# ZechangSun/QFA

Hardware: AMD Instinct MI355X
Metric: spectra/sec per EM step (higher is better)
Workload: dtype f32

## Files before the change

### qfa_amd/csrc/qfa_common.h

```cpp
#pragma once
#include <hip/hip_runtime.h>
#include <stdint.h>

#include <type_traits>
#include <utility>

#include "../../include/qfa_hip.h"

typedef float f32x4 __attribute__((ext_vector_type(4)));

#define QFA_LOG2PI 1.8378770664093453f
#define QFA_LOG2E 1.4426950408889634f
#define QFA_LN2 0.6931471805599453f

template <int KP>
struct Cfg {
    static constexpr int FW = KP < 16 ? 16 : KP;
    static constexpr int KK2 = KP * (KP + 1) / 2;
    static constexpr int NT = (KK2 + 15) / 16;
    static constexpr int PW = NT * 16;
    static constexpr int NFT = FW / 16;
    static constexpr int PFT_PSI = KP + KK2;
    static constexpr int NR = (KP + KK2 + 5 + 3) / 4 * 4;
    static constexpr bool XS3 = KP == 16 || KP == 32;
    static constexpr int PFT_MAIN = XS3 ? (NR * 16 + 255) / 256 * 256 : NR * 16;
    static constexpr int PFT_FP = XS3 ? (KP == 32 ? 1536 : 512) : 0;
    static constexpr int PFT_F16H = 768, PFT_F16M = 1024, PFT_F16IT = 1280;
    static constexpr int TILE_PFT = PFT_MAIN + PFT_FP;
    static constexpr int NMOM = 2 * PW + 2 * FW + 4;
    static constexpr int MOM_T = PW, MOM_B = 2 * PW, MOM_B2 = 2 * PW + FW, MOM_S = 2 * PW + 2 * FW;
    static constexpr int NSOL = 2 * KP + KK2 + KP * KP;
    static constexpr int SOL_CI = KP, SOL_Z = KP + KK2, SOL_P = KP + KK2 + KP * KP;
};

__host__ __device__ constexpr int pair_index(int a, int b, int KP) {
    return a * KP - (a * (a - 1)) / 2 + (b - a);
}

__host__ __device__ inline int round_up(int x, int m) { return (x + m - 1) / m * m; }

#ifndef QFA_PX_SPW
#define QFA_PX_SPW 2
#endif
#ifndef QFA_PX_SPW8
#define QFA_PX_SPW8 1
#endif
struct WorkPlan {
    int full, rem, nseg, seg_tiles;
    __host__ __device__ int items() const { return full + rem * nseg; }
};
__device__ __forceinline__ void plan_item(const WorkPlan &w, int item, int ntiles, int &blk, int &seg, int &t0,
                                          int &t1) {
    if (item < w.full) {
        blk = item; seg = 0; t0 = 0; t1 = ntiles;
    } else {
        const int j = item - w.full;
        blk = w.full + j % w.rem;
        seg = j / w.rem;
        t0 = seg * w.seg_tiles;
        t1 = min(t0 + w.seg_tiles, ntiles);
    }
}

template <int NMOM>
__device__ __forceinline__ float *mom_segment(float *MOM, const WorkPlan &w, int seg, int Bpad, int spb = 64) {
    if (seg == 0) return MOM;
    const size_t row0 = (size_t)w.full * spb, R = (size_t)Bpad - row0;
    return MOM + ((size_t)Bpad + (size_t)(seg - 1) * R - row0) * NMOM;
}

struct Scal64 {
    double s[3];
    unsigned ticket, pad;
};
__device__ __forceinline__ void scal64_commit(Scal64 *q, double a, double b, double c, unsigned nwaves, float *accS) {
    if ((threadIdx.x & 63) != 0) return;
    if (a != 0.0) atomicAdd(&q->s[0], a);
    if (b != 0.0) atomicAdd(&q->s[1], b);
    if (c != 0.0) atomicAdd(&q->s[2], c);
    __threadfence();
    if (atomicAdd(&q->ticket, 1u) == nwaves - 1u) {
        __threadfence();
        accS[0] += (float)__hip_atomic_load(&q->s[0], __ATOMIC_RELAXED, __HIP_MEMORY_SCOPE_AGENT);
        accS[1] += (float)__hip_atomic_load(&q->s[1], __ATOMIC_RELAXED, __HIP_MEMORY_SCOPE_AGENT);
        accS[2] += (float)__hip_atomic_load(&q->s[2], __ATOMIC_RELAXED, __HIP_MEMORY_SCOPE_AGENT);
    }
}

struct DevConsts {
    float tau0, c0, beta;
    float t_amp, t_lscale, t_expo, t_off;
    float offp, k1, omc0;
};

#ifdef QFA_PRECISE_MATH
__device__ __forceinline__ float fast_exp2(float x) { return exp2f(x); }
__device__ __forceinline__ float fast_log2(float x) { return log2f(x); }
__device__ __forceinline__ float fast_rcp(float x) { return 1.0f / x; }
#else
__device__ __forceinline__ float fast_exp2(float x) { return __builtin_amdgcn_exp2f(x); }
__device__ __forceinline__ float fast_log2(float x) { return __builtin_amdgcn_logf(x); }
__device__ __forceinline__ float fast_rcp(float x) { return __builtin_amdgcn_rcpf(x); }
#endif
__device__ __forceinline__ float fast_exp(float x) { return fast_exp2(x * QFA_LOG2E); }
__device__ __forceinline__ float fast_log(float x) { return fast_log2(x) * QFA_LN2; }

struct BlueTerms {
    float A, zd, pw, l2;
};

__device__ __forceinline__ BlueTerms blue_terms(float z, const DevConsts &k) {
    BlueTerms t;
    t.l2 = fast_log2(1.0f + z);
    float tau = k.t_amp * fast_exp2(k.t_expo * (t.l2 + k.t_lscale)) + k.t_off;
    t.A = fast_exp(-tau);
    t.pw = fast_exp2(k.beta * t.l2);
    float re = 1.0f - k.c0 - fast_exp(-k.tau0 * t.pw);
    t.zd = re * re;
    return t;
}

struct ZFac {
    float ts, pw, l2;
};
__device__ __forceinline__ ZFac zfac_load(const float4 *__restrict__ ZS, int s, bool valid) {
    ZFac z{0.f, 0.f, 0.f};
    if (valid) {
        const float4 q = ZS[s];
        z.ts = q.x; z.pw = q.y; z.l2 = q.z;
    }
    return z;
}
__device__ __forceinline__ BlueTerms blue_terms_zf(const ZFac &zs, float ti, float pwi, float l2i, const DevConsts &k) {
    BlueTerms t;
    t.l2 = zs.l2 + l2i;
    t.pw = zs.pw * pwi;
    t.A = fast_exp2(fmaf(zs.ts, ti, k.offp));
    const float re = k.omc0 - fast_exp2(k.k1 * t.pw);
    t.zd = re * re;
    return t;
}
__device__ __forceinline__ unsigned long long batch_row(const qfa_batch_t &bt, int s) {
    return bt.rows ? (unsigned long long)(unsigned)bt.rows[s] : (unsigned long long)(unsigned)s;
}
template <int SH>
__device__ __forceinline__ const unsigned char *lane_ptr(const void *sbase, unsigned long long off) {
    return reinterpret_cast<const unsigned char *>(sbase) + (off << SH);
}

__device__ __forceinline__ float4 zfac_spec(float zq1, float beta, const qfa_tau_t &tau) {
    const double l2s = log2((double)zq1);
    const double ts = -1.4426950408889634 * (double)tau.amp * exp2((double)tau.expo * (l2s + log2((double)tau.scale)));
    return float4{(float)ts, (float)exp2((double)beta * l2s), (float)l2s, 0.f};
}
__device__ __forceinline__ void zfac_spec_body(int s, const float *__restrict__ zq1, const int *__restrict__ rows,
                                               const qfa_params_t &p, const qfa_tau_t &tau, int B, float4 *__restrict__ ZS) {
    if (s >= B) return;
    ZS[s] = zfac_spec(zq1[rows ? rows[s] : s], *p.beta, tau);
}
static __global__ void k_zfac_spec(const float *__restrict__ zq1, const int *__restrict__ rows, qfa_params_t p, qfa_tau_t tau,
                                   int B, float4 *__restrict__ ZS) {
    zfac_spec_body(blockIdx.x * blockDim.x + threadIdx.x, zq1, rows, p, tau, B, ZS);
}
static __global__ void k_zfac_pix(const float *__restrict__ pix_ratio, qfa_params_t p, qfa_tau_t tau, int Nb,
                                  float4 *__restrict__ ZP) {
    const int i = blockIdx.x * blockDim.x + threadIdx.x;
    if (i >= Nb) return;
    const double l2i = log2((double)pix_ratio[i]);
    ZP[i] = float4{(float)exp2((double)tau.expo * l2i), (float)exp2((double)*p.beta * l2i), (float)l2i, 0.f};
}

struct ZPSrc {
    const float4 *tab;
    const float *ratio;
    const float *beta;
    float expo;
    float offp;
    __device__ __forceinline__ bool on() const { return tab != nullptr || ratio != nullptr; }
    __device__ __forceinline__ float4 at(int i) const {
        if (tab) return tab[i];
        const double l2i = log2((double)ratio[i]);
        return float4{(float)exp2((double)expo * l2i), (float)exp2((double)*beta * l2i), (float)l2i, 0.f};
    }
};
__host__ __device__ inline ZPSrc zp_table(const float4 *ZP, float offp = 0.f) { return ZPSrc{ZP, nullptr, nullptr, 0.f, offp}; }

__device__ __forceinline__ f32x4 mfma4(float a, float b, f32x4 c) {
    return __builtin_amdgcn_mfma_f32_16x16x4f32(a, b, c, 0, 0, 0);
}


typedef unsigned u32x4 __attribute__((ext_vector_type(4)));
typedef unsigned u32x2 __attribute__((ext_vector_type(2)));
typedef __bf16 bf16x8 __attribute__((ext_vector_type(8)));
typedef short s16x4 __attribute__((ext_vector_type(4)));

typedef __bf16 bf16x2 __attribute__((ext_vector_type(2)));
typedef float f32x2v __attribute__((ext_vector_type(2)));
__device__ __forceinline__ unsigned cvt_pk_bf16(float a, float b) {
    return __builtin_bit_cast(unsigned, __builtin_convertvector(f32x2v{a, b}, bf16x2));
}
__device__ __forceinline__ unsigned split_c_lo() {
    unsigned c;
    asm("s_mov_b32 %0, 0xbf80" : "=s"(c));
    return c;
}
__device__ __forceinline__ unsigned split_c_hi() {
    unsigned c;
    asm("s_mov_b32 %0, 0xbf800000" : "=s"(c));
    return c;
}
__device__ __forceinline__ float sub_bf16_lo(float x, unsigned packed) {
    return __builtin_amdgcn_fdot2_f32_bf16(__builtin_bit_cast(bf16x2, packed), __builtin_bit_cast(bf16x2, split_c_lo()), x, false);
}
__device__ __forceinline__ float sub_bf16_hi(float x, unsigned packed) {
    return __builtin_amdgcn_fdot2_f32_bf16(__builtin_bit_cast(bf16x2, packed), __builtin_bit_cast(bf16x2, split_c_hi()), x, false);
}
__device__ __forceinline__ void split2(float x0, float x1, unsigned &h, unsigned &m, unsigned &l) {
    h = cvt_pk_bf16(x0, x1);
    const float r0 = sub_bf16_lo(x0, h), r1 = sub_bf16_hi(x1, h);
    m = cvt_pk_bf16(r0, r1);
    const float s0 = sub_bf16_lo(r0, m), s1 = sub_bf16_hi(r1, m);
    l = cvt_pk_bf16(s0, s1);
}
__device__ __forceinline__ void split8(const float (&x)[8], u32x4 &h, u32x4 &m, u32x4 &l) {
#pragma unroll
    for (int q = 0; q < 4; ++q) {
        unsigned a, b, c;
        split2(x[2 * q], x[2 * q + 1], a, b, c);
        h[q] = a; m[q] = b; l[q] = c;
    }
}
__device__ __forceinline__ f32x4 xdl(const u32x4 &a, const u32x4 &b, f32x4 c) {
    return __builtin_amdgcn_mfma_f32_16x16x32_bf16(__builtin_bit_cast(bf16x8, a), __builtin_bit_cast(bf16x8, b), c, 0,
                                                   0, 0);
}
typedef _Float16 f16x8 __attribute__((ext_vector_type(8)));
typedef _Float16 f16x2 __attribute__((ext_vector_type(2)));
__device__ __forceinline__ void split2h(float x0, float x1, unsigned &h, unsigned &m) {
    const _Float16 h0 = (_Float16)x0, h1 = (_Float16)x1;
    const _Float16 m0 = (_Float16)(x0 - (float)h0), m1 = (_Float16)(x1 - (float)h1);
    h = __builtin_bit_cast(unsigned, f16x2{h0, h1});
    m = __builtin_bit_cast(unsigned, f16x2{m0, m1});
}
__device__ __forceinline__ void split8h(const float (&x)[8], u32x4 &h, u32x4 &m) {
#pragma unroll
    for (int q = 0; q < 4; ++q) {
        unsigned a, b;
        split2h(x[2 * q], x[2 * q + 1], a, b);
        h[q] = a; m[q] = b;
    }
}
__device__ __forceinline__ f32x4 xdlh(const u32x4 &a, const u32x4 &b, f32x4 c) {
    return __builtin_amdgcn_mfma_f32_16x16x32_f16(__builtin_bit_cast(f16x8, a), __builtin_bit_cast(f16x8, b), c, 0, 0, 0);
}
__device__ __forceinline__ f32x4 xdl3h(const u32x4 &ah, const u32x4 &am, const u32x4 &bh, const u32x4 &bm, f32x4 c) {
    c = xdlh(ah, bm, c);
    c = xdlh(am, bh, c);
    return xdlh(ah, bh, c);
}
__host__ __device__ __forceinline__ float f16_row_scale(float amax, float &inv) {
    int e = 0;
    if (amax > 0.f && amax < 3.0e38f) (void)frexpf(amax, &e); else e = 14;
    e = e < -100 ? -100 : (e > 100 ? 100 : e);
    inv = ldexpf(1.f, e - 14);
    return ldexpf(1.f, 14 - e);
}
__host__ __device__ __forceinline__ float f16_weight_scale(float psi) {
    if (!(psi > 0.f && psi < 3.0e38f)) return 0.015625f;
    int e = 0;
    (void)frexpf(psi, &e);
    e = e < -60 ? -60 : (e > 60 ? 60 : e);
    return ldexpf(1.f, 11 + e);
}
__device__ __forceinline__ f32x4 xdl16(const u32x2 &a, const u32x2 &b, f32x4 c) {
    return __builtin_amdgcn_mfma_f32_16x16x16bf16_1k(__builtin_bit_cast(s16x4, a), __builtin_bit_cast(s16x4, b), c, 0,
                                                     0, 0);
}
template <typename V, typename F>
__device__ __forceinline__ f32x4 six_terms(F &&mm, const V &ah, const V &am, const V &al, const V &bh, const V &bm,
                                           const V &bl, f32x4 c) {
    c = mm(ah, bl, c);
    c = mm(al, bh, c);
    c = mm(am, bm, c);
    c = mm(am, bh, c);
    c = mm(ah, bm, c);
    return mm(ah, bh, c);
}
__device__ __forceinline__ f32x4 xdl6(const u32x4 &ah, const u32x4 &am, const u32x4 &al, const u32x4 &bh,
                                      const u32x4 &bm, const u32x4 &bl, f32x4 c) {
    return six_terms([](const u32x4 &a, const u32x4 &b, f32x4 cc) { return xdl(a, b, cc); }, ah, am, al, bh, bm, bl, c);
}
__device__ __forceinline__ f32x4 xdl16_6(const u32x2 &ah, const u32x2 &am, const u32x2 &al, const u32x2 &bh,
                                         const u32x2 &bm, const u32x2 &bl, f32x4 c) {
    return six_terms([](const u32x2 &a, const u32x2 &b, f32x4 cc) { return xdl16(a, b, cc); }, ah, am, al, bh, bm, bl, c);
}

__device__ __forceinline__ void glds16(const void *g, void *lds_base) {
    __builtin_amdgcn_global_load_lds((const __attribute__((address_space(1))) void *)g,
                                     (__attribute__((address_space(3))) void *)lds_base, 16, 0, 0);
}

__device__ __forceinline__ void pin(float &x) { asm volatile("" : "+v"(x)); }
template <typename... T>
__device__ __forceinline__ void pin(float &x, T &...rest) {
    pin(x);
    pin(rest...);
}

__device__ __forceinline__ int dpp_row_bcast(int v, int l) {
#define QFA_BC(n) case n: return __builtin_amdgcn_mov_dpp(v, 0x150 + n, 0xf, 0xf, true);
    switch (l & 15) {
        QFA_BC(0) QFA_BC(1) QFA_BC(2) QFA_BC(3) QFA_BC(4) QFA_BC(5) QFA_BC(6) QFA_BC(7)
        QFA_BC(8) QFA_BC(9) QFA_BC(10) QFA_BC(11) QFA_BC(12) QFA_BC(13) QFA_BC(14) QFA_BC(15)
    }
#undef QFA_BC
    return v;
}
__device__ __forceinline__ int half_bcast(int v, int l) {
    const int a = __builtin_amdgcn_readlane(v, l & 31), b = __builtin_amdgcn_readlane(v, 32 + (l & 31));
    return (threadIdx.x & 32) ? b : a;
}
template <int KP>
__device__ __forceinline__ float group_bcast(float x, int l) {
    if constexpr (KP == 16) return __int_as_float(dpp_row_bcast(__float_as_int(x), l));
    else if constexpr (KP == 32) return __int_as_float(half_bcast(__float_as_int(x), l));
    else return __shfl(x, l, KP);
}
template <int KP>
__device__ __forceinline__ double group_bcast(double x, int l) {
    if constexpr (KP == 16) {
        const int lo = dpp_row_bcast(__double2loint(x), l), hi = dpp_row_bcast(__double2hiint(x), l);
        return __hiloint2double(hi, lo);
    } else if constexpr (KP == 32) {
        const int lo = half_bcast(__double2loint(x), l), hi = half_bcast(__double2hiint(x), l);
        return __hiloint2double(hi, lo);
    } else {
        return __shfl(x, l, KP);
    }
}

template <typename F, int... I>
__device__ __forceinline__ void static_for_impl(F &&f, std::integer_sequence<int, I...>) {
    (f(std::integral_constant<int, I>{}), ...);
}
template <int N, typename F>
__device__ __forceinline__ void static_for(F &&f) {
    static_for_impl(f, std::make_integer_sequence<int, N>{});
}

__device__ __forceinline__ int wave_uniform(int x) { return __builtin_amdgcn_readfirstlane(x); }

__device__ __forceinline__ DevConsts load_consts(const qfa_params_t &p, const qfa_tau_t &tau) {
    DevConsts k;
    k.tau0 = *p.tau0;
    k.c0 = *p.c0;
    k.beta = *p.beta;
    const double l2s = log2((double)tau.scale);
    k.t_lscale = (float)l2s;
    k.t_amp = (float)((double)tau.amp * exp2((double)tau.expo * (l2s - (double)k.t_lscale)));
    k.t_expo = tau.expo;
    k.t_off = tau.offset;
    k.offp = -QFA_LOG2E * k.t_off;
    k.k1 = -QFA_LOG2E * k.tau0;
    k.omc0 = 1.0f - k.c0;
    return k;
}
```

### qfa_amd/csrc/qfa_step_kernels.h

```cpp
#pragma once
#include <type_traits>

#include "qfa_common.h"
#include "qfa_gt_layout.h"

template <int KP>
__global__ void k_prep_pft(const float *__restrict__ F, const float *__restrict__ Psi,
                           const float *__restrict__ omega, const float4 *__restrict__ ZP, int Npix, int Nb, int Nh,
                           int NpixPad, float *__restrict__ PFT) {
    using C = Cfg<KP>;
    const int i = blockIdx.x * blockDim.y + threadIdx.y;
    if (i >= NpixPad) return;
    const bool live = i < Npix;
    float *pft = PFT + (size_t)(i >> 4) * C::TILE_PFT + (i & 15);
    for (int r = threadIdx.x; r < C::NR; r += blockDim.x) {
        float v = 0.f;
        if (r < KP) {
            if (live && r < Nh) v = F[(size_t)i * Nh + r];
        } else if (r < C::PFT_PSI) {
            const int pidx = r - KP;
            int a = 0;
            while (a + 1 < KP && pair_index(a + 1, a + 1, KP) <= pidx) ++a;
            const int b = a + (pidx - pair_index(a, a, KP));
            if (live && b < Nh) v = F[(size_t)i * Nh + a] * F[(size_t)i * Nh + b];
        } else if (r == C::PFT_PSI) {
            if (live) v = Psi[i];
        } else if (r == C::PFT_PSI + 1) {
            if (i < Nb) v = omega[i];
        } else if (ZP && i < Nb && r < C::PFT_PSI + 5) {
            const float4 q = ZP[i];
            v = r == C::PFT_PSI + 2 ? q.x : (r == C::PFT_PSI + 3 ? q.y : q.z);
        }
        pft[r * 16] = v;
    }
    if constexpr (C::XS3 && KP == 32) {
        if (threadIdx.x < 4) {
            const int g = threadIdx.x;
            unsigned *fp = reinterpret_cast<unsigned *>(PFT + (size_t)(i >> 4) * C::TILE_PFT + C::PFT_MAIN) +
                           (g * 16 + (i & 15)) * 4;
#pragma unroll
            for (int q = 0; q < 4; ++q) {
                const int a = 8 * g + 2 * q;
                const float v0 = (live && a < Nh) ? F[(size_t)i * Nh + a] : 0.f;
                const float v1 = (live && a + 1 < Nh) ? F[(size_t)i * Nh + a + 1] : 0.f;
                unsigned h, m, l;
                split2(v0, v1, h, m, l);
                fp[q] = h; fp[256 + q] = m; fp[512 + q] = l;
            }
            float mx = 0.f, x[8];
#pragma unroll
            for (int j = 0; j < 8; ++j) {
                x[j] = (live && 8 * g + j < Nh) ? F[(size_t)i * Nh + 8 * g + j] : 0.f;
                mx = fmaxf(mx, fabsf(x[j]));
            }
            mx = fmaxf(mx, __shfl_xor(mx, 1));
            mx = fmaxf(mx, __shfl_xor(mx, 2));
            float it;
            const float t = f16_row_scale(mx, it);
#pragma unroll
            for (int j = 0; j < 8; ++j) x[j] *= t;
            u32x4 h4, m4;
            split8h(x, h4, m4);
#pragma unroll
            for (int q = 0; q < 4; ++q) { fp[C::PFT_F16H + q] = h4[q]; fp[C::PFT_F16M + q] = m4[q]; }
            if (g == 0) reinterpret_cast<float *>(PFT + (size_t)(i >> 4) * C::TILE_PFT + C::PFT_MAIN)[C::PFT_F16IT + (i & 15)] = it;
        }
    } else if constexpr (C::XS3) {
        if (threadIdx.x < 4) {
            const int g = threadIdx.x;
            float v[4];
#pragma unroll
            for (int j = 0; j < 4; ++j) v[j] = (live && 4 * g + j < Nh) ? F[(size_t)i * Nh + 4 * g + j] : 0.f;
            unsigned h0, m0, l0, h1, m1, l1;
            split2(v[0], v[1], h0, m0, l0);
            split2(v[2], v[3], h1, m1, l1);
            unsigned *fp = reinterpret_cast<unsigned *>(PFT + (size_t)(i >> 4) * C::TILE_PFT + C::PFT_MAIN) +
                           g * 32 + (i & 15) * 2;
            fp[0] = h0; fp[1] = h1;
            fp[128] = m0; fp[129] = m1;
            fp[256] = l0; fp[257] = l1;
        }
    }
}

struct __attribute__((packed, aligned(4))) f4u { float v[4]; };
struct __attribute__((packed, aligned(1))) u4u { unsigned char v[4]; };

static __global__ void k_sum_segments(float4 *__restrict__ mom, const float4 *__restrict__ rest, int nseg, size_t n4) {
    const size_t i = (size_t)blockIdx.x * blockDim.x + threadIdx.x;
    if (i >= n4) return;
    float4 a = mom[i];
    for (int g = 1; g < nseg; ++g) {
        const float4 b = rest[(size_t)(g - 1) * n4 + i];
        a.x += b.x; a.y += b.y; a.z += b.z; a.w += b.w;
    }
    mom[i] = a;
}

template <int KP, bool PREDICT, bool STATE = false, bool NLLRED = false>
__global__ __launch_bounds__(256, KP <= 16 ? 4 : 2) void k_solve(const float *__restrict__ MOM, float *__restrict__ SOL,
                                               float *__restrict__ nll_out, float *__restrict__ nblue_out, int B,
                                               int Nh, float *__restrict__ hmean, float *__restrict__ hcov,
                                               unsigned *__restrict__ ticket = nullptr,
                                               unsigned char *__restrict__ PST = nullptr, float *__restrict__ scal = nullptr,
                                               int exact = 0) {
    static_assert(!NLLRED || (!PREDICT && !STATE), "NLLRED: the training step of a small batch");
    using C = Cfg<KP>;
    constexpr int G = 64 / KP;
    static_assert(!STATE || ((KP == 16 || KP == 8) && !PREDICT), "state images: N_h <= 16, training step");
    __shared__ __attribute__((aligned(16))) float s_rows[STATE ? 4 * G * C::NSOL : 1];
    if (ticket && blockIdx.x == 0 && threadIdx.x == 0) {
        *ticket = 0u;
        Scal64 *q = reinterpret_cast<Scal64 *>(ticket + 2);
        q->s[0] = 0.0; q->s[1] = 0.0; q->s[2] = 0.0; q->ticket = 0u;
    }
    const int lane = threadIdx.x & 63;
    const int c = lane % KP;
    const int s = (blockIdx.x * (blockDim.x >> 6) + (threadIdx.x >> 6)) * G + lane / KP;
    const bool valid = s < B;
    const float *mom = MOM + (size_t)(valid ? s : B - 1) * C::NMOM;

    constexpr bool VIA_LDS = KP == 32;
    __shared__ __attribute__((aligned(16))) double s_col[VIA_LDS ? 4 * G * KP : 1];
    __shared__ __attribute__((aligned(16))) float s_T[VIA_LDS ? 4 * G * KP * KP : 1];
    double *col = s_col + ((threadIdx.x >> 6) * G + lane / KP) * (VIA_LDS ? KP : 0);
    auto wave_lds_sync = [&]() {
        asm volatile("s_waitcnt lgkmcnt(0)" ::: "memory");
        __builtin_amdgcn_wave_barrier();
    };

    double Cc[KP];
    static_for<KP>([&](auto R) {
        constexpr int r = decltype(R)::value;
        const int a = r < c ? r : c, b = r < c ? c : r;
        Cc[r] = (double)mom[pair_index(a, b, KP)] + (r == c ? 1.0 : 0.0);
    });
    double logdet = 0.0, pprod = 1.0;
    static_for<KP>([&](auto JJ) {
        constexpr int jj = decltype(JJ)::value;
        if constexpr (VIA_LDS) {
            if (c == jj) static_for<KP>([&](auto R) { col[decltype(R)::value] = Cc[decltype(R)::value]; });
            wave_lds_sync();
        }
        const double piv = VIA_LDS ? col[jj] : group_bcast<KP>(Cc[jj], jj);
        pprod *= piv;
        if ((jj & 7) == 7 || jj == KP - 1) {
            logdet += log(pprod);
            pprod = 1.0;
        }
        const double ip = 1.0 / piv;
        const double rjc = (c == jj) ? ip : Cc[jj] * ip;
        const double keep = (c == jj) ? 0.0 : 1.0;
        static_for<KP>([&](auto I) {
            constexpr int i = decltype(I)::value;
            if constexpr (i != jj) {
                const double cij = VIA_LDS ? col[i] : group_bcast<KP>(Cc[i], jj);
                Cc[i] = fma(-cij, rjc, Cc[i] * keep);
            }
        });
        Cc[jj] = rjc;
        if constexpr (VIA_LDS) wave_lds_sync();
        __builtin_amdgcn_sched_barrier(0);
    });
    const double bc = (double)mom[C::MOM_B + c];
    double y = 0.0;
    if constexpr (VIA_LDS) {
        col[c] = bc;
        wave_lds_sync();
    }
    static_for<KP>([&](auto R) {
        constexpr int r = decltype(R)::value;
        y += Cc[r] * (VIA_LDS ? col[r] : group_bcast<KP>(bc, r));
    });
    double quad = bc * y;
#pragma unroll
    for (int o = KP / 2; o >= 1; o >>= 1) quad += __shfl_xor(quad, o, KP);
    const float *sc = mom + C::MOM_S;
    const double nll = 0.5 * ((double)sc[0] - quad + (double)sc[2] * (double)QFA_LOG2PI + (double)sc[1] + logdet);
    if (valid && c == 0) {
        nll_out[s] = (float)nll;
        if (nblue_out) nblue_out[s] = sc[3];
    }

    float *sol = STATE ? s_rows + ((threadIdx.x >> 6) * G + lane / KP) * C::NSOL : SOL + (size_t)(valid ? s : 0) * C::NSOL;
    if (valid) {
        sol[c] = (float)y;
        static_for<KP>([&](auto R) {
            constexpr int r = decltype(R)::value;
            if (r <= c) sol[C::SOL_CI + pair_index(r, c, KP)] = (float)(r == c ? Cc[r] : 2.0 * Cc[r]);
        });
    }
    if (PREDICT) {
        if (valid && c < Nh) {
            hmean[(size_t)s * Nh + c] = (float)y;
            static_for<KP>([&](auto R) {
                constexpr int r = decltype(R)::value;
                if (r < Nh) hcov[((size_t)s * Nh + c) * Nh + r] = (float)Cc[r];
            });
        }
        return;
    }
    float Zr[KP];
    double pc;
    if (exact) {
        static_for<KP>([&](auto Bq) { Zr[decltype(Bq)::value] = -(float)Cc[decltype(Bq)::value]; });
        pc = y;
    } else {
    float Tc[KP];
    const float *momT = mom;
    if constexpr (VIA_LDS) asm volatile("" : "+v"(momT));
    static_for<KP>([&](auto R) {
        constexpr int r = decltype(R)::value;
        const int a = r < c ? r : c, b = r < c ? c : r;
        Tc[r] = momT[C::MOM_T + pair_index(a, b, KP)];
    });
    static_for<KP>([&](auto Bq) { Zr[decltype(Bq)::value] = 0.f; });
    pc = (double)mom[C::MOM_B2 + c];
    if constexpr (VIA_LDS) {
        float *Tl = s_T + ((threadIdx.x >> 6) * G + lane / KP) * KP * KP;
        wave_lds_sync();
        static_for<KP>([&](auto M) { Tl[decltype(M)::value * KP + c] = Tc[decltype(M)::value]; });
        col[c] = y;
        wave_lds_sync();
        static_for<KP>([&](auto M) {
            constexpr int m = decltype(M)::value;
            pc -= (double)Tc[m] * col[m];
        });
        __builtin_amdgcn_sched_barrier(0);
        static_for<KP>([&](auto M) {
            constexpr int m = decltype(M)::value;
            const float cm = (float)Cc[m];
            static_for<KP / 4>([&](auto Bq) {
                constexpr int b = 4 * decltype(Bq)::value;
                const float4 t = *reinterpret_cast<const float4 *>(Tl + m * KP + b);
                Zr[b] = fmaf(cm, t.x, Zr[b]);
                Zr[b + 1] = fmaf(cm, t.y, Zr[b + 1]);
                Zr[b + 2] = fmaf(cm, t.z, Zr[b + 2]);
                Zr[b + 3] = fmaf(cm, t.w, Zr[b + 3]);
            });
            static_for<KP>([&](auto Bq) { pin(Zr[decltype(Bq)::value]); });
            asm volatile("" ::: "memory");
            __builtin_amdgcn_sched_barrier(0);
        });
    } else {
        static_for<KP>([&](auto M) {
            constexpr int m = decltype(M)::value;
            const float cm = (float)Cc[m];
            static_for<KP>([&](auto Bq) {
                constexpr int b = decltype(Bq)::value;
                Zr[b] = fmaf(cm, group_bcast<KP>(Tc[m], b), Zr[b]);
            });
            static_for<KP>([&](auto Bq) { pin(Zr[decltype(Bq)::value]); });
            __builtin_amdgcn_sched_barrier(0);
        });
    }
    if constexpr (!VIA_LDS) {
        static_for<KP>([&](auto M) {
            constexpr int m = decltype(M)::value;
            pc -= (double)Tc[m] * group_bcast<KP>(y, m);
        });
    }
    }
    if (valid) {
        static_for<KP>([&](auto Bq) {
            constexpr int b = decltype(Bq)::value;
            sol[C::SOL_Z + c * KP + b] = Zr[b];
        });
        sol[C::SOL_P + c] = (float)pc;
    }
    if constexpr (STATE) {
        __syncthreads();
#pragma unroll
        for (int q = 0; q < (4 * G) / 16; ++q) {
            const int grp = (int)blockIdx.x * ((4 * G) / 16) + q;
            if (16 * grp < B)
                build_state<KP>(s_rows + q * 16 * C::NSOL, 16 * grp, B, Nh, PST + (size_t)grp * GTT<KP>::STATE_B, (int)threadIdx.x);
        }
    }
    if constexpr (NLLRED) {
        __shared__ double sh[2][4];
        __shared__ bool last;
        __threadfence();
        __syncthreads();
        if (threadIdx.x == 0) last = atomicAdd(ticket + 1, 1u) == (unsigned)gridDim.x - 1u;
        __syncthreads();
        if (!last) return;
        __threadfence();
        double a = 0.0, nb = 0.0;
        for (int q = threadIdx.x; q < B; q += 256) {
            a += (double)__hip_atomic_load(nll_out + q, __ATOMIC_RELAXED, __HIP_MEMORY_SCOPE_AGENT);
            nb += __hip_atomic_load(nblue_out + q, __ATOMIC_RELAXED, __HIP_MEMORY_SCOPE_AGENT) > 0.f ? 1.0 : 0.0;
        }
        for (int o = 32; o >= 1; o >>= 1) {
            a += __shfl_xor(a, o);
            nb += __shfl_xor(nb, o);
        }
        const int w = threadIdx.x >> 6;
        if ((threadIdx.x & 63) == 0) { sh[0][w] = a; sh[1][w] = nb; }
        __syncthreads();
        if (threadIdx.x == 0) {
            double ta = 0.0, tb = 0.0;
            for (int i = 0; i < 4; ++i) { ta += sh[0][i]; tb += sh[1][i]; }
            scal[3] += (float)tb;
            scal[4] += (float)ta;
            scal[5] += (float)B;
            if (exact) scal[6] += (float)B;
        }
    }
}

constexpr int NRED = 32;
static __global__ __launch_bounds__(256) void k_reduce_nll(const float *__restrict__ nll, const float *__restrict__ nblue,
                                                           int B, float *__restrict__ scal, double *__restrict__ part,
                                                           unsigned *__restrict__ ticket, int exact) {
    __shared__ double sh[2][4];
    __shared__ bool last;
    const int per = (B + (int)gridDim.x - 1) / (int)gridDim.x, s0 = blockIdx.x * per, s1 = min(B, s0 + per);
    double a = 0.0, nb = 0.0;
    for (int s = s0 + threadIdx.x; s < s1; s += 256) {
        a += (double)nll[s];
        nb += nblue[s] > 0.f ? 1.0 : 0.0;
    }
    for (int o = 32; o >= 1; o >>= 1) {
        a += __shfl_xor(a, o);
        nb += __shfl_xor(nb, o);
    }
    const int w = threadIdx.x >> 6;
    if ((threadIdx.x & 63) == 0) { sh[0][w] = a; sh[1][w] = nb; }
    __syncthreads();
    if (threadIdx.x == 0) {
        double ta = 0.0, tb = 0.0;
        for (int i = 0; i < 4; ++i) { ta += sh[0][i]; tb += sh[1][i]; }
        part[blockIdx.x] = ta;
        part[NRED + blockIdx.x] = tb;
        __threadfence();
        last = atomicAdd(ticket, 1u) == (unsigned)gridDim.x - 1u;
        if (last) {
            __threadfence();
            ta = 0.0; tb = 0.0;
            for (int i = 0; i < (int)gridDim.x; ++i) {
                ta += __hip_atomic_load(part + i, __ATOMIC_RELAXED, __HIP_MEMORY_SCOPE_AGENT);
                tb += __hip_atomic_load(part + NRED + i, __ATOMIC_RELAXED, __HIP_MEMORY_SCOPE_AGENT);
            }
            scal[3] += (float)tb;
            scal[4] += (float)ta;
            scal[5] += (float)B;
            if (exact) scal[6] += (float)B;
        }
    }
}

struct SpecRegs2 {
    float d[4], sg[4], z[4];
    unsigned m[4];
};

#ifndef QFA_G8_OCC
#define QFA_G8_OCC 2
#endif
struct PixPar {
    float Psi, om, ti, pwi, l2i;
};
template <int KP, bool HASA, bool ZF, bool EXACT>
__global__ __launch_bounds__(256, KP == 8 ? QFA_G8_OCC : 2) void k_grads(qfa_params_t p, qfa_batch_t bt, qfa_tau_t tau, int B,
                                                              int Npix, int Nb, int Nh, int ntiles, WorkPlan wp,
                                                              const float *__restrict__ PFT,
                                                              const float *__restrict__ SOL,
                                                              float *__restrict__ accum, float *__restrict__ slab,
                                                              double *__restrict__ slabS, int slab_stride,
                                                              Scal64 *__restrict__ sc64, const float4 *__restrict__ ZS) {
    static_assert(KP == 8 || KP == 16, "k_grads: N_h <= 16 (N_h = 17..32 runs k_s12_x + k_grads_s3)");
    using C = Cfg<KP>;
    constexpr int KF = KP / 4, KQ = C::KK2 / 4;
    constexpr int NF4 = C::TILE_PFT / 4;
    constexpr int NPART = 512;
    constexpr bool XS3 = KP == 16;
    constexpr int NM4 = C::PFT_MAIN / 4, NP4 = XS3 ? C::PFT_FP / 4 : 1, RING_M = XS3 ? 2 : 3;
    constexpr int NCH_MAIN = C::PFT_MAIN / 256, NCH = C::TILE_PFT / 256;
    __shared__ float4 lds4[RING_M][XS3 ? NM4 : NF4];
    __shared__ float4 ldsfp[XS3 ? 3 : 1][NP4];
    __shared__ unsigned ldszl[XS3 ? 4 : 1][XS3 ? 16 * 64 * 2 : 1];
    __shared__ float ldspart[2][4][NPART];
    const int tid = threadIdx.x;
    const int lane = tid & 63;
    const int wv = wave_uniform(tid >> 6);
    int blk, seg, t0, t1;
    plan_item(wp, blockIdx.x, ntiles, blk, seg, t0, t1);
    const int s0 = (blk * 4 + wv) * 16;
    const bool active = s0 < B;
    const int nbt = (Nb + 15) >> 4;
    for (int i = tid; i < 2 * 4 * NPART; i += 256) (&ldspart[0][0][0])[i] = 0.f;
    const DevConsts k = load_consts(p, tau);
    const int lo = lane & 15, g = lane >> 4;

    const bool det = slab != nullptr;
    float *accF = det ? slab + (size_t)blk * (size_t)slab_stride : accum;
    float *accA = accF + (size_t)Npix * Nh;
    float *accS = accum + (size_t)Npix * Nh + 3 * (size_t)Npix + Nb;
    auto add_to = [&](float *q, float v) {
        if (det) *q = v;
        else atomicAdd(q, v);
    };

    float yA[KF], qA[KQ];
    {
        const bool v = active && (s0 + lo) < B;
        const float *sol = SOL + (size_t)(v ? s0 + lo : 0) * C::NSOL;
#pragma unroll
        for (int t = 0; t < KF; ++t) yA[t] = v ? sol[4 * t + g] : 0.f;
#pragma unroll
        for (int t = 0; t < KQ; ++t) qA[t] = v ? sol[C::SOL_CI + 4 * t + g] : 0.f;
    }
    constexpr int NZR = XS3 ? 1 : 4, NZA = XS3 ? 1 : KP, NZS = XS3 ? 16 : 1;
    float Zr[NZR][NZA], pr[4];
    u32x2 Zh[NZS], Zm[NZS];
    u32x2 ph = {0u, 0u}, pm = {0u, 0u}, pl = {0u, 0u};
    bool sv[4];
    unsigned rowi[4];
    int offB[4];
#pragma unroll
    for (int r = 0; r < 4; ++r) {
        const int srel = 4 * g + r;
        sv[r] = active && (s0 + srel) < B;
        const bool v = sv[r] && lo < KP;
        const float *sol = SOL + (size_t)(v ? s0 + srel : 0) * C::NSOL;
        if constexpr (!XS3) {
#pragma unroll
            for (int a = 0; a < KP; ++a) Zr[r][a] = v ? sol[C::SOL_Z + a * KP + lo] : 0.f;
        }
        pr[r] = v ? sol[C::SOL_P + lo] : 0.f;
        const int sc = active ? min(srel, B - 1 - s0) : 0;
        rowi[r] = (unsigned)batch_row(bt, (active ? s0 : 0) + sc);
        offB[r] = sc * Nb;
    }
    if constexpr (XS3) {
        unsigned *zl = ldszl[wv];
        float zraw[16][4];
#pragma unroll
        for (int s = 0; s < 16; ++s) {
            const bool v = active && (s0 + s) < B;
            const float *sol = SOL + (size_t)(v ? s0 + s : 0) * C::NSOL + C::SOL_Z + lo;
#pragma unroll
            for (int j = 0; j < 4; ++j) zraw[s][j] = v ? sol[(4 * g + j) * KP] : 0.f;
        }
        __builtin_amdgcn_sched_barrier(0);
#pragma unroll
        for (int s = 0; s < 16; ++s) {
            const float *z = zraw[s];
            unsigned h0, m0, l0, h1, m1, l1;
            split2(z[0], z[1], h0, m0, l0);
            split2(z[2], z[3], h1, m1, l1);
            Zh[s] = u32x2{h0, h1};
            Zm[s] = u32x2{m0, m1};
            zl[(s * 64 + lane) * 2] = l0;
            zl[(s * 64 + lane) * 2 + 1] = l1;
        }
        unsigned h0, m0, l0, h1, m1, l1;
        split2(pr[0], pr[1], h0, m0, l0);
        split2(pr[2], pr[3], h1, m1, l1);
        ph = u32x2{h0, h1}; pm = u32x2{m0, m1}; pl = u32x2{l0, l1};
    }
    const float *abase = bt.A_blue ? bt.A_blue + (size_t)(active ? s0 : 0) * Nb : nullptr;
    ZFac zs[4];
#pragma unroll
    for (int r = 0; r < 4; ++r) zs[r] = zfac_load(ZS, s0 + 4 * g + r, ZF && sv[r]);
    const float4 *PFT4 = reinterpret_cast<const float4 *>(PFT);
    static_assert(XS3 || NF4 <= 256, "KP = 8: one staging register per thread holds the tile");
    float4 tv = {0.f, 0.f, 0.f, 0.f};
    double s_tau0 = 0.0, s_c0 = 0.0, s_beta = 0.0;
    int ntile_done = 0;

    auto run = [&](auto blue_tag, int ta, int tb) {
        constexpr bool BLUE = decltype(blue_tag)::value;
        const int n = tb - ta;
        if (n <= 0) return;
        const int rot = (int)(((unsigned)blk * 2654435761u) % (unsigned)min(n, 64));
        auto tile_of = [&](int c) {
            int x = c + rot;
            if (x >= n) x -= n;
            return ta + x;
        };

        auto load_spec = [&](int tg, SpecRegs2 &rg) {
            const unsigned px = (unsigned)min(16 * tg + lo, Npix - 1);
#pragma unroll
            for (int r = 0; r < 4; ++r) {
                unsigned ri = rowi[r];
                asm volatile("" : "+v"(ri));
                const unsigned long long o = (unsigned long long)ri * (unsigned long long)bt.row_stride + px;
                rg.d[r] = bt.delta[o];
                rg.sg[r] = bt.error[o];
                rg.m[r] = bt.mask[o];
            }
            if (BLUE && !ZF) {
                const unsigned pz = (unsigned)min(16 * tg + lo, Nb - 1);
#pragma unroll
                for (int r = 0; r < 4; ++r) {
                    unsigned ri = rowi[r];
                    asm volatile("" : "+v"(ri));
                    rg.z[r] = bt.zabs[(unsigned long long)ri * (unsigned)Nb + pz];
                }
            }
        };

        auto read_pix = [&](const float *tile, PixPar &pp) {
            pp.Psi = tile[C::PFT_PSI * 16 + lo];
            pp.om = tile[(C::PFT_PSI + 1) * 16 + lo];
            if (BLUE && ZF) {
                pp.ti = tile[(C::PFT_PSI + 2) * 16 + lo];
                pp.pwi = tile[(C::PFT_PSI + 3) * 16 + lo];
                pp.l2i = tile[(C::PFT_PSI + 4) * 16 + lo];
            }
        };
        auto stage1 = [&](const float *tile, f32x4 &afy, f32x4 &aq, PixPar &pp) {
            constexpr int NK1 = KF + KQ;
            const float *tb_ = tile + g * 16 + lo;
            f32x4 a0 = {0.f, 0.f, 0.f, 0.f}, a1 = {0.f, 0.f, 0.f, 0.f}, a2 = {0.f, 0.f, 0.f, 0.f};
#pragma unroll
            for (int t = 0; t < NK1; ++t) {
                const int row = t < KF ? 4 * t : KP + 4 * (t - KF);
                const float bv = tb_[row * 16];
                if (t < KF) a0 = mfma4(yA[t], bv, a0);
                else if (t & 1) a1 = mfma4(qA[t - KF], bv, a1);
                else a2 = mfma4(qA[t - KF], bv, a2);
            }
            afy = a0;
            aq = a1 + a2;
            read_pix(tile, pp);
        };

        auto region1 = [&](int tg, const SpecRegs2 &cur, const f32x4 &afy, const f32x4 &aq, const PixPar &pp,
                           const float *tileN, f32x4 &afyN, f32x4 &aqN, PixPar &ppN,
                           float (&betaR)[4], float (&gamR)[4], float *part) {
            constexpr int NK1 = KF + KQ, AHEAD = 6;
            const float *tbN = tileN + g * 16 + lo;
            f32x4 a0 = {0.f, 0.f, 0.f, 0.f}, a1 = {0.f, 0.f, 0.f, 0.f}, a2 = {0.f, 0.f, 0.f, 0.f};
            float bop[8];
            auto rd = [&](int t) {
                if (t < NK1) bop[t & 7] = tbN[(t < KF ? 4 * t : KP + 4 * (t - KF)) * 16];
            };
            auto mf = [&](int t) {
                if (t < KF) a0 = mfma4(yA[t < KF ? t : 0], bop[t & 7], a0);
                else if (t < NK1 && (t & 1)) a1 = mfma4(qA[t < NK1 ? t - KF : 0], bop[t & 7], a1);
                else if (t < NK1) a2 = mfma4(qA[t < NK1 ? t - KF : 0], bop[t & 7], a2);
            };
            int slot_no = 0;
            auto slots = [&](int nslot) {
#pragma unroll
                for (int i = 0; i < nslot; ++i) {
                    rd(slot_no + AHEAD);
                    mf(slot_no);
                    ++slot_no;
                }
                __builtin_amdgcn_sched_barrier(0);
            };
#pragma unroll
            for (int t = 0; t < AHEAD; ++t) rd(t);
            read_pix(tileN, ppN);
            __builtin_amdgcn_sched_barrier(0);
            const float Psi = pp.Psi, om = pp.om;

            const int px = 16 * tg + lo;
            const bool inb = px < Npix;
            const bool blue = px < Nb;
            float gPsi = 0.f, gOm = 0.f, sA = 0.f, cnt = 0.f;
            float t_tau0 = 0.f, t_c0 = 0.f, t_beta = 0.f;
            float dd[4], l2[4], x1[4], x2[4], pw[4], y1[4], y2[4], Av[4], zd[4], A2[4], wD[4], wDA[4], uu[4], dG[4];
            float rex[4], exv[4];
            bool wv_[4];
#pragma unroll
            for (int r = 0; r < 4; ++r) {
                dd[r] = cur.d[r];
                wv_[r] = inb & sv[r] & (cur.m[r] != 0);
            }
#pragma unroll
            for (int rp = 0; rp < 4; rp += 2) {
                if (BLUE) {
#pragma unroll
                    for (int r = rp; r < rp + 2; ++r) {
                        if (ZF) {
                            l2[r] = zs[r].l2 + pp.l2i;
                            pw[r] = zs[r].pw * pp.pwi;
                            pin(l2[r], pw[r]);
                        } else {
                            l2[r] = fast_log2(1.0f + cur.z[r]);
                            x1[r] = k.t_expo * (l2[r] + k.t_lscale);
                            x2[r] = k.beta * l2[r];
                            pin(x1[r], x2[r]);
                        }
                    }
                    slots(2);
#pragma unroll
                    for (int r = rp; r < rp + 2; ++r) {
                        if (ZF) {
                            y1[r] = fmaf(zs[r].ts, pp.ti, k.offp);
                            y2[r] = k.k1 * pw[r];
                        } else {
                            pw[r] = fast_exp2(x2[r]);
                            const float tauv = k.t_amp * fast_exp2(x1[r]) + k.t_off;
                            y1[r] = -tauv * QFA_LOG2E;
                            y2[r] = -k.tau0 * pw[r] * QFA_LOG2E;
                        }
                        pin(y1[r], y2[r]);
                    }
                    slots(2);
#pragma unroll
                    for (int r = rp; r < rp + 2; ++r) {
                        float Ab = fast_exp2(y1[r]);
                        if (HASA) Ab = abase[offB[r] + min(px, Nb - 1)];
                        const float ex = fast_exp2(y2[r]);
                        const float re = 1.0f - k.c0 - ex;
                        Av[r] = blue ? Ab : 1.f;
                        zd[r] = blue ? re * re : 0.f;
                        rex[r] = blue ? re : 0.f;
                        exv[r] = ex;
                        pin(Av[r], zd[r]);
                    }
                    slots(2);
#pragma unroll
                    for (int r = rp; r < rp + 2; ++r) {
                        A2[r] = Av[r] * Av[r];
                        const float D = A2[r] * Psi + om * zd[r] + cur.sg[r] * cur.sg[r];
                        wD[r] = wv_[r] ? fast_rcp(D) : 0.f;
                        dd[r] = wv_[r] ? dd[r] : 0.f;
                        wDA[r] = wD[r] * Av[r];
                        pin(wDA[r], dd[r]);
                    }
                    slots(4);
#pragma unroll
                    for (int r = rp; r < rp + 2; ++r) {
                        uu[r] = wD[r] * (dd[r] - Av[r] * afy[r]);
                        const float dS = wD[r] - wDA[r] * wDA[r] * aq[r];
                        dG[r] = 0.5f * (dS - uu[r] * uu[r]);
                        gPsi += A2[r] * dG[r];
                        gOm += dG[r] * zd[r];
                    }
                    pin(gPsi, gOm);
                    slots(4);
#pragma unroll
                    for (int r = rp; r < rp + 2; ++r) {
                        const float root = 1.0f - k.tau0 * pw[r] - k.c0;
                        const float er = dG[r] * (om * zd[r]) * zd[r] * 2.0f * root;
                        const float ee = dG[r] * om * 2.0f * rex[r];
                        const float e = EXACT ? ee : er, et = EXACT ? -ee * exv[r] : er;
                        t_tau0 -= et * pw[r];
                        t_beta -= et * (k.tau0 * pw[r] * (l2[r] * QFA_LN2));
                        t_c0 -= e;
                    }
                    pin(t_tau0, t_beta, t_c0);
                    slots(4);
#pragma unroll
                    for (int r = rp; r < rp + 2; ++r) {
                        cnt += wv_[r] ? 1.f : 0.f;
                        betaR[r] = wDA[r] * Av[r];
                        sA += betaR[r] * Av[r];
                        gamR[r] = Av[r] * uu[r];
                        pin(gamR[r]);
                    }
                    pin(cnt, sA);
                    slots(2);
                } else {
#pragma unroll
                    for (int r = rp; r < rp + 2; ++r) {
                        const float D = Psi + cur.sg[r] * cur.sg[r];
                        wD[r] = wv_[r] ? fast_rcp(D) : 0.f;
                        dd[r] = wv_[r] ? dd[r] : 0.f;
                        pin(wD[r], dd[r]);
                    }
                    slots(6);
#pragma unroll
                    for (int r = rp; r < rp + 2; ++r) {
                        uu[r] = wD[r] * (dd[r] - afy[r]);
                        const float dS = wD[r] - wD[r] * wD[r] * aq[r];
                        gPsi += 0.5f * (dS - uu[r] * uu[r]);
                    }
                    pin(gPsi);
                    slots(6);
#pragma unroll
                    for (int r = rp; r < rp + 2; ++r) {
                        cnt += wv_[r] ? 1.f : 0.f;
                        betaR[r] = wD[r];
                        sA += wD[r];
                        gamR[r] = uu[r];
                        pin(gamR[r]);
                    }
                    pin(cnt, sA);
                    slots(8);
                }
            }
            static_assert(NK1 <= 40 && AHEAD < 8, "stage 1 has more K-steps than MFMA slots");
            if (BLUE) {
                s_tau0 += (double)t_tau0;
                s_c0 += (double)t_c0;
                s_beta += (double)t_beta;
            }
            afyN = a0;
            aqN = a1 + a2;
            part[256 + lane] = sA;
            part[320 + lane] = gPsi;
            part[384 + lane] = gOm;
            part[448 + lane] = cnt;
        };

        auto stage3 = [&](const float *tile, const float (&betaR)[4], const float (&gamR)[4], float *part) {
          if constexpr (!XS3) {
            float f[KP];
#pragma unroll
            for (int a = 0; a < KP; ++a) f[a] = tile[a * 16 + lo];
            f32x4 aG = {0.f, 0.f, 0.f, 0.f}, aG2 = {0.f, 0.f, 0.f, 0.f};
#pragma unroll
            for (int r = 0; r < 4; ++r) {
#pragma unroll
                for (int a = 0; a < KP; a += 2) {
                    aG = mfma4(betaR[r] * f[a], Zr[r][a], aG);
                    aG2 = mfma4(betaR[r] * f[a + 1], Zr[r][a + 1], aG2);
                }
                if (r & 1) aG = mfma4(gamR[r], pr[r], aG);
                else aG2 = mfma4(gamR[r], pr[r], aG2);
            }
            aG += aG2;
#pragma unroll
            for (int rr = 0; rr < 4; ++rr) part[(4 * g + rr) * 16 + lo] = aG[rr];
          }
        };

        auto stage3x = [&](const float4 *fpt, const float (&betaR)[4], const float (&gamR)[4], float *part) {
            if constexpr (XS3) {
#pragma unroll
                for (int r = 0; r < 4; ++r) part[(4 * g + r) * 16 + lo] = betaR[r];
                const u32x2 *fp = reinterpret_cast<const u32x2 *>(fpt) + lane;
                const u32x2 Fh = fp[0], Fm = fp[64];
                unsigned h0, m0, l0, h1, m1, l1;
                split2(gamR[0], gamR[1], h0, m0, l0);
                split2(gamR[2], gamR[3], h1, m1, l1);
                const f32x4 zero = {0.f, 0.f, 0.f, 0.f};
                f32x4 acc = xdl16_6(u32x2{h0, h1}, u32x2{m0, m1}, u32x2{l0, l1}, ph, pm, pl, zero);
                const u32x2 *zl = reinterpret_cast<const u32x2 *>(ldszl[wv]) + lane;
                const float4 *brow = reinterpret_cast<const float4 *>(part) + g;
#pragma unroll
                for (int s = 0; s < 16; ++s) {
                    const f32x4 G = xdl16_6(Fh, Fm, fp[128], Zh[s], Zm[s], zl[s * 64], zero);
                    const float4 bq = brow[s * 4];
                    acc[0] = fmaf(bq.x, G[0], acc[0]);
                    acc[1] = fmaf(bq.y, G[1], acc[1]);
                    acc[2] = fmaf(bq.z, G[2], acc[2]);
                    acc[3] = fmaf(bq.w, G[3], acc[3]);
                }
#pragma unroll
                for (int rr = 0; rr < 4; ++rr) part[(4 * g + rr) * 16 + lo] = acc[rr];
            }
        };

        auto flush = [&](int tg, const float (*pp)[NPART], bool extra) {
            const int base = 16 * tg;
            {
                const int idx = lane + 64 * wv;
                const float v = (pp[0][idx] + pp[1][idx]) + (pp[2][idx] + pp[3][idx]);
                const int px = base + (idx >> 4), b = idx & 15;
                if ((b < Nh) & (px < Npix)) add_to(accF + (size_t)px * Nh + b, v);
            }
            if (extra) {
                const int which = lane >> 4, px = base + (lane & 15);
                float v = 0.f;
#pragma unroll
                for (int w = 0; w < 4; ++w) {
                    const float *q = pp[w] + 256 + which * 64 + (lane & 15);
                    v += (q[0] + q[16]) + (q[32] + q[48]);
                }
                const int off = which * Npix - (which == 3 ? Npix - Nb : 0) + px;
                const bool ok = (px < Npix) & ((which != 2) | (px < Nb));
                if (ok) add_to(accA + off, v);
            }
        };
        auto tilebuf = [&](int c) { return reinterpret_cast<const float *>(lds4[c % RING_M]); };
        auto get_tile = [&](int c) {
            if constexpr (XS3) {
                const unsigned char *src = reinterpret_cast<const unsigned char *>(PFT4 + (size_t)tile_of(c) * NF4) + lane * 16;
#pragma unroll
                for (int i = 0; i < (NCH + 3) / 4; ++i) {
                    const int ch = wv + 4 * i;
                    if (ch < NCH_MAIN) glds16(src + ch * 1024, reinterpret_cast<unsigned char *>(lds4[c % RING_M]) + ch * 1024);
                    else if (ch < NCH) glds16(src + ch * 1024, reinterpret_cast<unsigned char *>(ldsfp[c % 3]) + (ch - NCH_MAIN) * 1024);
                }
            } else {
                tv = PFT4[(size_t)tile_of(c) * NF4 + min(tid, NF4 - 1)];
            }
        };
        auto put_tile = [&](int c) {
            if constexpr (!XS3) {
                if (tid < NF4) lds4[c % RING_M][tid] = tv;
            }
        };

        f32x4 afy, aq;
        PixPar pxp{0.f, 0.f, 0.f, 0.f, 0.f};
        auto step = [&](int c, const SpecRegs2 &cur, SpecRegs2 &nxt) {
            const bool more = c + 1 < n;
            const int tg = tile_of(c);
            const int pbuf = c & 1;
            f32x4 afyN = {0.f, 0.f, 0.f, 0.f}, aqN = {0.f, 0.f, 0.f, 0.f};
            PixPar pxpN{0.f, 0.f, 0.f, 0.f, 0.f};
            float betaR[4] = {0.f, 0.f, 0.f, 0.f}, gamR[4] = {0.f, 0.f, 0.f, 0.f};
            if (active) {
                const int cn1 = more ? c + 1 : c;
                load_spec(tile_of(cn1), nxt);
                region1(tg, cur, afy, aq, pxp, tilebuf(cn1), afyN, aqN, pxpN, betaR, gamR,
                        ldspart[pbuf][wv]);
                __builtin_amdgcn_sched_barrier(0);
            }
            if (c + 2 < n) get_tile(c + 2);
            if (active) {
                if constexpr (XS3) stage3x(ldsfp[c % 3], betaR, gamR, ldspart[pbuf][wv]);
                else stage3(tilebuf(c), betaR, gamR, ldspart[pbuf][wv]);
                afy = afyN; aq = aqN; pxp = pxpN;
            }
            if (c + 2 < n) put_tile(c + 2);
            __syncthreads();
            flush(tg, ldspart[pbuf], wv == (ntile_done & 3));
            ++ntile_done;
        };

        SpecRegs2 ra, rb;
        get_tile(0);
        put_tile(0);
        if (n > 1) {
            get_tile(1);
            put_tile(1);
        }
        if (active) load_spec(tile_of(0), ra);
        __syncthreads();
        if (active) stage1(tilebuf(0), afy, aq, pxp);
        if constexpr (XS3) __syncthreads();
        for (int c = 0; c < n; c += 2) {
            step(c, ra, rb);
            if (c + 1 < n) step(c + 1, rb, ra);
        }
        __syncthreads();
    };
    run(std::true_type{}, t0, min(t1, nbt));
    run(std::false_type{}, max(t0, nbt), t1);

    if (!active) {
        if (det && lane == 0) {
            double *q = slabS + ((size_t)blockIdx.x * 4 + wv) * 3;
            q[0] = 0.0; q[1] = 0.0; q[2] = 0.0;
        } else if (!det) {
            scal64_commit(sc64, 0.0, 0.0, 0.0, gridDim.x * 4u, accS);
        }
        return;
    }
    for (int o = 32; o >= 1; o >>= 1) {
        s_tau0 += __shfl_xor(s_tau0, o);
        s_c0 += __shfl_xor(s_c0, o);
        s_beta += __shfl_xor(s_beta, o);
    }
    if (lane == 0) {
        if (det) {
            double *q = slabS + ((size_t)blockIdx.x * 4 + wv) * 3;
            q[0] = s_tau0; q[1] = s_c0; q[2] = s_beta;
        } else {
            scal64_commit(sc64, s_tau0, s_c0, s_beta, gridDim.x * 4u, accS);
        }
    }
}

#ifndef QFA_DET_CHUNK_ROWS
#define QFA_DET_CHUNK_ROWS 32
#endif
static __global__ __launch_bounds__(256) void k_reduce_slab_rows(const float *__restrict__ slab, int nblk, size_t NF,
                                                                 size_t stride, double *__restrict__ part) {
    const size_t j = (size_t)blockIdx.x * 256 + threadIdx.x;
    if (j >= NF) return;
    const int r0 = blockIdx.y * QFA_DET_CHUNK_ROWS, r1 = min(nblk, r0 + QFA_DET_CHUNK_ROWS);
    const float *q = slab + (size_t)r0 * stride + j;
    double a = 0.0;
    int r = r0;
    for (; r + 8 <= r1; r += 8, q += 8 * stride) {
        const float v0 = q[0], v1 = q[stride], v2 = q[2 * stride], v3 = q[3 * stride], v4 = q[4 * stride],
                    v5 = q[5 * stride], v6 = q[6 * stride], v7 = q[7 * stride];
        a += (double)v0; a += (double)v1; a += (double)v2; a += (double)v3;
        a += (double)v4; a += (double)v5; a += (double)v6; a += (double)v7;
    }
    for (; r < r1; ++r, q += stride) a += (double)q[0];
    part[(size_t)blockIdx.y * NF + j] = a;
}
static __global__ __launch_bounds__(256) void k_reduce_slab_fin(const double *__restrict__ part,
                                                                const double *__restrict__ slabS, int nch,
                                                                int nitemwaves, size_t NF, float *__restrict__ accum) {
    const size_t j = (size_t)blockIdx.x * 256 + threadIdx.x;
    if (j < NF) {
        double a = 0.0;
        for (int c = 0; c < nch; ++c) a += part[(size_t)c * NF + j];
        accum[j] += (float)a;
    }
    __shared__ double sh[3][256];
    if (blockIdx.x == 0) {
        const int per = (nitemwaves + 255) / 256, q0 = threadIdx.x * per, q1 = min(nitemwaves, q0 + per);
        double a0 = 0.0, a1 = 0.0, a2 = 0.0;
        for (int q = q0; q < q1; ++q) {
            a0 += slabS[(size_t)q * 3 + 0];
            a1 += slabS[(size_t)q * 3 + 1];
            a2 += slabS[(size_t)q * 3 + 2];
        }
        sh[0][threadIdx.x] = a0; sh[1][threadIdx.x] = a1; sh[2][threadIdx.x] = a2;
        __syncthreads();
        if (threadIdx.x < 3) {
            double a = 0.0;
            for (int t = 0; t < 256; ++t) a += sh[threadIdx.x][t];
            accum[NF + threadIdx.x] += (float)a;
        }
    }
}

template <int KP>
__global__ __launch_bounds__(256) void k_predict_out(const float *__restrict__ mu, int B, int Npix, int ntiles,
                                                     const float *__restrict__ PFT, const float *__restrict__ SOL,
                                                     float *__restrict__ cont, float *__restrict__ unc) {
    using C = Cfg<KP>;
    constexpr int KF = KP / 4, KQ = C::KK2 / 4;
    const int lane = threadIdx.x & 63;
    const int s0 = (blockIdx.x * (blockDim.x >> 6) + (threadIdx.x >> 6)) * 16;
    if (s0 >= B) return;
    const int lo = lane & 15, g = lane >> 4;
    float yA[KF], qA[KQ];
    {
        const bool v = (s0 + lo) < B;
        const float *sol = SOL + (size_t)(v ? s0 + lo : 0) * C::NSOL;
#pragma unroll
        for (int t = 0; t < KF; ++t) yA[t] = v ? sol[4 * t + g] : 0.f;
#pragma unroll
        for (int t = 0; t < KQ; ++t) qA[t] = v ? sol[C::SOL_CI + 4 * t + g] : 0.f;
    }
    for (int tg = 0; tg < ntiles; ++tg) {
        const int px = 16 * tg + lo;
        f32x4 afy = {0.f, 0.f, 0.f, 0.f}, aq = {0.f, 0.f, 0.f, 0.f};
        const float *tb = PFT + (size_t)tg * C::TILE_PFT + g * 16 + lo;
#pragma unroll
        for (int t = 0; t < KF; ++t) afy = mfma4(yA[t], tb[(4 * t) * 16], afy);
#pragma unroll
        for (int t = 0; t < KQ; ++t) aq = mfma4(qA[t], tb[(KP + 4 * t) * 16], aq);
        if (px < Npix) {
            const float m = mu[px];
#pragma unroll
            for (int r = 0; r < 4; ++r) {
                const int s = s0 + 4 * g + r;
                if (s < B) {
                    cont[(size_t)s * Npix + px] = afy[r] + m;
                    unc[(size_t)s * Npix + px] = __builtin_amdgcn_sqrtf(aq[r]);
                }
            }
        }
    }
}
```

Baseline: 34.14 million.

## Replace Gauss-Jordan inversion with Cholesky plus triangular-inverse product for small KP

```diff
diff --git a/qfa_amd/csrc/qfa_common.h b/qfa_amd/csrc/qfa_common.h
--- a/qfa_amd/csrc/qfa_common.h
+++ b/qfa_amd/csrc/qfa_common.h
@@ -317,6 +317,15 @@
 #undef QFA_BC
     return v;
 }
+__device__ __forceinline__ double dpp_row_bcast(double v, int l) {
+#define QFA_BC(n) case n: return __builtin_amdgcn_update_dpp(0.0, v, 0x150 + n, 0xf, 0xf, true);
+    switch (l & 15) {
+        QFA_BC(0) QFA_BC(1) QFA_BC(2) QFA_BC(3) QFA_BC(4) QFA_BC(5) QFA_BC(6) QFA_BC(7)
+        QFA_BC(8) QFA_BC(9) QFA_BC(10) QFA_BC(11) QFA_BC(12) QFA_BC(13) QFA_BC(14) QFA_BC(15)
+    }
+#undef QFA_BC
+    return v;
+}
 __device__ __forceinline__ int half_bcast(int v, int l) {
     const int a = __builtin_amdgcn_readlane(v, l & 31), b = __builtin_amdgcn_readlane(v, 32 + (l & 31));
     return (threadIdx.x & 32) ? b : a;
@@ -330,8 +339,7 @@
 template <int KP>
 __device__ __forceinline__ double group_bcast(double x, int l) {
     if constexpr (KP == 16) {
-        const int lo = dpp_row_bcast(__double2loint(x), l), hi = dpp_row_bcast(__double2hiint(x), l);
-        return __hiloint2double(hi, lo);
+        return dpp_row_bcast(x, l);
     } else if constexpr (KP == 32) {
         const int lo = half_bcast(__double2loint(x), l), hi = half_bcast(__double2hiint(x), l);
         return __hiloint2double(hi, lo);
diff --git a/qfa_amd/csrc/qfa_step_kernels.h b/qfa_amd/csrc/qfa_step_kernels.h
--- a/qfa_amd/csrc/qfa_step_kernels.h
+++ b/qfa_amd/csrc/qfa_step_kernels.h
@@ -97,6 +97,12 @@
     mom[i] = a;
 }
 
+__device__ __forceinline__ double rsqrt_refined(double d) {
+    const double s0 = __builtin_amdgcn_rsq(d);
+    const double e = fma(-(d * s0), s0, 1.0);
+    return fma(s0 * e, fma(e, 0.375, 0.5), s0);
+}
+
 template <int KP, bool PREDICT, bool STATE = false, bool NLLRED = false>
 __global__ __launch_bounds__(256, KP <= 16 ? 4 : 2) void k_solve(const float *__restrict__ MOM, float *__restrict__ SOL,
                                                float *__restrict__ nll_out, float *__restrict__ nblue_out, int B,
@@ -136,13 +142,46 @@
         Cc[r] = (double)mom[pair_index(a, b, KP)] + (r == c ? 1.0 : 0.0);
     });
     double logdet = 0.0, pprod = 1.0;
+    if constexpr (!VIA_LDS) {
+        double Xc[KP];
+        static_for<KP>([&](auto R) { Xc[decltype(R)::value] = decltype(R)::value == c ? 1.0 : 0.0; });
+        static_for<KP>([&](auto JJ) {
+            constexpr int jj = decltype(JJ)::value;
+            const double piv = group_bcast<KP>(Cc[jj], jj);
+            pprod *= piv;
+            if ((jj & 7) == 7 || jj == KP - 1) {
+                logdet += log(pprod);
+                pprod = 1.0;
+            }
+            const double s = rsqrt_refined(piv);
+            const double lj = Cc[jj] * s, xj = Xc[jj] * s;
+            Xc[jj] = xj;
+            static_for<KP>([&](auto K) {
+                constexpr int k = decltype(K)::value;
+                if constexpr (k > jj) {
+                    const double lkj = group_bcast<KP>(lj, k);
+                    Cc[k] = fma(-lkj, lj, Cc[k]);
+                    Xc[k] = fma(-lkj, xj, Xc[k]);
+                }
+            });
+            __builtin_amdgcn_sched_barrier(0);
+        });
+        static_for<KP>([&](auto K) {
+            constexpr int k = decltype(K)::value;
+            double a = Xc[k] * group_bcast<KP>(Xc[k], k);
+            static_for<KP>([&](auto M) {
+                constexpr int m = decltype(M)::value;
+                if constexpr (m > k) a = fma(Xc[m], group_bcast<KP>(Xc[m], k), a);
+            });
+            Cc[k] = a;
+        });
+        __builtin_amdgcn_sched_barrier(0);
+    } else {
     static_for<KP>([&](auto JJ) {
         constexpr int jj = decltype(JJ)::value;
-        if constexpr (VIA_LDS) {
-            if (c == jj) static_for<KP>([&](auto R) { col[decltype(R)::value] = Cc[decltype(R)::value]; });
-            wave_lds_sync();
-        }
-        const double piv = VIA_LDS ? col[jj] : group_bcast<KP>(Cc[jj], jj);
+        if (c == jj) static_for<KP>([&](auto R) { col[decltype(R)::value] = Cc[decltype(R)::value]; });
+        wave_lds_sync();
+        const double piv = col[jj];
         pprod *= piv;
         if ((jj & 7) == 7 || jj == KP - 1) {
             logdet += log(pprod);
@@ -154,14 +193,15 @@
         static_for<KP>([&](auto I) {
             constexpr int i = decltype(I)::value;
             if constexpr (i != jj) {
-                const double cij = VIA_LDS ? col[i] : group_bcast<KP>(Cc[i], jj);
+                const double cij = col[i];
                 Cc[i] = fma(-cij, rjc, Cc[i] * keep);
             }
         });
         Cc[jj] = rjc;
-        if constexpr (VIA_LDS) wave_lds_sync();
+        wave_lds_sync();
         __builtin_amdgcn_sched_barrier(0);
     });
+    }
     const double bc = (double)mom[C::MOM_B + c];
     double y = 0.0;
     if constexpr (VIA_LDS) {
```

Measured after the change: 34.29 million, median of 6. About the same (+0.5%).
